# tyui592/Real_Time_Helmet_Detection

Hardware: AMD Instinct MI355X
Metric: train imgs/sec (higher is better)
Workload: dtype bf16; 1 GPU; model=hourglass-1-ch128, global_batch=16, imsize=512, parallelism=dp1, engine=hip, fp8=False, hipgraph=True

## Files before the change

### real_time_helmet_detection_amd/ops/csrc/bindings.cpp

```cpp
#include <torch/extension.h>

namespace rthd {
torch::Tensor add_act_fwd(torch::Tensor a, torch::Tensor b, int64_t act);
torch::Tensor add_act_bwd(torch::Tensor dy, torch::Tensor y, int64_t act);

std::vector<torch::Tensor> pool2x2_fwd(torch::Tensor x, bool is_max,
                                       bool need_arg);
torch::Tensor pool2x2_bwd(torch::Tensor dy, torch::Tensor arg, bool is_max,
                          int64_t H, int64_t W);
std::vector<torch::Tensor> maxpool_same_fwd(torch::Tensor x, int64_t k,
                                            bool need_arg);
torch::Tensor maxpool_same_bwd(torch::Tensor dy, torch::Tensor arg,
                               int64_t k);

torch::Tensor upsample2x_add_fwd(torch::Tensor x,
                                 c10::optional<torch::Tensor> skip);
torch::Tensor upsample2x_bwd(torch::Tensor dy);

std::vector<torch::Tensor> centernet_loss_fwd(
    torch::Tensor phm, torch::Tensor poff, torch::Tensor psize,
    torch::Tensor ghm, torch::Tensor goff, torch::Tensor gsize,
    torch::Tensor mask, double alpha, double beta);
std::vector<torch::Tensor> centernet_loss_bwd(
    torch::Tensor phm, torch::Tensor poff, torch::Tensor psize,
    torch::Tensor ghm, torch::Tensor goff, torch::Tensor gsize,
    torch::Tensor mask, torch::Tensor sums, torch::Tensor gout,
    double alpha, double beta);
std::vector<torch::Tensor> centernet_loss_fused_fwd(
    torch::Tensor out, torch::Tensor ghm, torch::Tensor goff,
    torch::Tensor gsize, torch::Tensor mask, double alpha, double beta,
    bool sig_os);
torch::Tensor centernet_loss_fused_bwd(
    torch::Tensor out, torch::Tensor ghm, torch::Tensor goff,
    torch::Tensor gsize, torch::Tensor mask, torch::Tensor sums,
    torch::Tensor glosses, double alpha, double beta, bool sig_os);

std::vector<torch::Tensor> decode_fwd(torch::Tensor hm, torch::Tensor off,
                                      torch::Tensor wh, int64_t scale_factor,
                                      int64_t topk, int64_t pool_size,
                                      bool normalized);
std::vector<torch::Tensor> decode_logits(torch::Tensor out,
                                         int64_t scale_factor, int64_t topk,
                                         int64_t pool_size, bool normalized,
                                         bool flip);
torch::Tensor nms_fwd(torch::Tensor boxes, torch::Tensor scores,
                      double iou_threshold);
std::vector<torch::Tensor> nms_batched(torch::Tensor boxes,
                                       torch::Tensor scores,
                                       double iou_threshold,
                                       double conf_th);
std::vector<torch::Tensor> soft_nms_fwd(torch::Tensor boxes,
                                        torch::Tensor scores, double sigma,
                                        double score_th);
std::vector<torch::Tensor> soft_nms_batched(torch::Tensor boxes,
                                            torch::Tensor scores,
                                            double sigma, double score_th,
                                            double conf_th);

torch::Tensor pack_weights(torch::Tensor w, bool swap, bool to_bf16);
std::vector<torch::Tensor> pack_weights_pair(torch::Tensor w,
                                             bool to_bf16_fwd,
                                             bool to_bf16_dgrad);
torch::Tensor pack_weights_fp8(torch::Tensor w);
torch::Tensor conv_fwd_fp8r(torch::Tensor x, torch::Tensor wpk,
                            torch::Tensor scale, torch::Tensor shift,
                            c10::optional<torch::Tensor> skip,
                            int64_t KH, int64_t KW, int64_t stride,
                            int64_t pad, int64_t Cout, int64_t act,
                            bool out_fp8);
torch::Tensor conv_fwd(torch::Tensor x, torch::Tensor wpk,
                       torch::Tensor scale, torch::Tensor shift,
                       c10::optional<torch::Tensor> skip,
                       int64_t KH, int64_t KW, int64_t stride, int64_t pad,
                       int64_t Cout, int64_t act);
torch::Tensor conv_fwd_small(torch::Tensor x, torch::Tensor wpk,
                             torch::Tensor scale, torch::Tensor shift,
                             c10::optional<torch::Tensor> skip,
                             int64_t KH, int64_t KW, int64_t stride,
                             int64_t pad, int64_t Cout, int64_t act,
                             int64_t splitk);
torch::Tensor conv_fwd_k64(torch::Tensor x, torch::Tensor wpk,
                           torch::Tensor scale, torch::Tensor shift,
                           c10::optional<torch::Tensor> skip,
                           int64_t KH, int64_t KW, int64_t stride,
                           int64_t pad, int64_t Cout, int64_t act);
torch::Tensor conv_fwd_halo(torch::Tensor x, torch::Tensor wpk,
                            torch::Tensor scale, torch::Tensor shift,
                            c10::optional<torch::Tensor> skip,
                            int64_t KH, int64_t KW, int64_t stride,
                            int64_t pad, int64_t Cout, int64_t act);
torch::Tensor stem_im2col(torch::Tensor x, int64_t KS, int64_t stride,
                          int64_t pad);
torch::Tensor wgrad(torch::Tensor x, torch::Tensor dy, int64_t KH,
                    int64_t KW, int64_t stride, int64_t pad);
torch::Tensor wgrad_bf16_fast(torch::Tensor x, torch::Tensor dy, int64_t KH,
                              int64_t KW, int64_t stride, int64_t pad,
                              const std::string& variant);
torch::Tensor lds_tr16_selftest();
std::string wgrad_bf16_choice(int64_t Cin, int64_t Cout, int64_t M);
int64_t wgrad_bf16_chunk_len(int64_t Cin, int64_t Cout, int64_t taps,
                             int64_t M);

std::vector<torch::Tensor> conv_fwd_stats(
    torch::Tensor x, torch::Tensor wpk, torch::Tensor scale,
    torch::Tensor shift, int64_t KH, int64_t KW, int64_t stride,
    int64_t pad, int64_t Cout, int64_t act);
std::vector<torch::Tensor> bn_stats_from_parts(
    torch::Tensor p1, torch::Tensor p2,
    c10::optional<torch::Tensor> running_mean,
    c10::optional<torch::Tensor> running_var,
    double momentum, double eps, int64_t M);
std::vector<torch::Tensor> bn_stats(torch::Tensor x,
                                    c10::optional<torch::Tensor> running_mean,
                                    c10::optional<torch::Tensor> running_var,
                                    double momentum, double eps);
torch::Tensor bn_act_fwd(torch::Tensor x, torch::Tensor mean,
                         torch::Tensor rstd, torch::Tensor gamma,
                         torch::Tensor beta, int64_t act,
                         c10::optional<torch::Tensor> skip);
std::vector<torch::Tensor> bn_act_bwd(torch::Tensor dy, torch::Tensor x,
                                      torch::Tensor mean, torch::Tensor rstd,
                                      torch::Tensor gamma, torch::Tensor beta,
                                      int64_t act,
                                      c10::optional<torch::Tensor> skip);
torch::Tensor col_sum(torch::Tensor x);

std::vector<torch::Tensor> encode_targets(torch::Tensor boxes,
                                          torch::Tensor labels, int64_t H,
                                          int64_t W, int64_t scale_factor,
                                          int64_t num_cls, bool normalized);
torch::Tensor normalize_u8(torch::Tensor img_u8, torch::Tensor table);
int64_t encode_chunk();
torch::Tensor augment_u8(torch::Tensor img_u8, torch::Tensor sizes,
                         torch::Tensor coef, int64_t T,
                         c10::optional<torch::Tensor> table);
}

PYBIND11_MODULE(TORCH_EXTENSION_NAME, m) {
  m.def("add_act_fwd", &rthd::add_act_fwd);
  m.def("add_act_bwd", &rthd::add_act_bwd);
  m.def("pool2x2_fwd", &rthd::pool2x2_fwd);
  m.def("pool2x2_bwd", &rthd::pool2x2_bwd);
  m.def("maxpool_same_fwd", &rthd::maxpool_same_fwd);
  m.def("maxpool_same_bwd", &rthd::maxpool_same_bwd);
  m.def("upsample2x_add_fwd", &rthd::upsample2x_add_fwd);
  m.def("upsample2x_bwd", &rthd::upsample2x_bwd);
  m.def("centernet_loss_fwd", &rthd::centernet_loss_fwd);
  m.def("centernet_loss_bwd", &rthd::centernet_loss_bwd);
  m.def("centernet_loss_fused_fwd", &rthd::centernet_loss_fused_fwd);
  m.def("centernet_loss_fused_bwd", &rthd::centernet_loss_fused_bwd);
  m.def("decode_fwd", &rthd::decode_fwd);
  m.def("decode_logits", &rthd::decode_logits);
  m.def("nms_fwd", &rthd::nms_fwd);
  m.def("nms_batched", &rthd::nms_batched);
  m.def("soft_nms", &rthd::soft_nms_fwd);
  m.def("soft_nms_batched", &rthd::soft_nms_batched);
  m.def("pack_weights",&rthd::pack_weights);
  m.def("pack_weights_pair", &rthd::pack_weights_pair);
  m.def("pack_weights_fp8", &rthd::pack_weights_fp8);
  m.def("conv_fwd_fp8r", &rthd::conv_fwd_fp8r);
  m.def("conv_fwd", &rthd::conv_fwd);
  m.def("conv_fwd_small", &rthd::conv_fwd_small);
  m.def("conv_fwd_k64", &rthd::conv_fwd_k64);
  m.def("conv_fwd_halo", &rthd::conv_fwd_halo);
  m.def("stem_im2col", &rthd::stem_im2col);
  m.def("wgrad", &rthd::wgrad);
  m.def("wgrad_bf16_fast", &rthd::wgrad_bf16_fast,
        py::arg("x"), py::arg("dy"), py::arg("kh"), py::arg("kw"),
        py::arg("stride"), py::arg("pad"), py::arg("variant") = "");
  m.def("lds_tr16_selftest", &rthd::lds_tr16_selftest);
  m.def("wgrad_bf16_choice", &rthd::wgrad_bf16_choice);
  m.def("wgrad_bf16_chunk_len", &rthd::wgrad_bf16_chunk_len);
  m.def("conv_fwd_stats", &rthd::conv_fwd_stats);
  m.def("bn_stats_from_parts", &rthd::bn_stats_from_parts,
        py::arg("p1"), py::arg("p2"), py::arg("running_mean") = py::none(),
        py::arg("running_var") = py::none(), py::arg("momentum") = 0.1,
        py::arg("eps") = 1e-5, py::arg("m") = 1);
  m.def("bn_stats", &rthd::bn_stats);
  m.def("bn_act_fwd", &rthd::bn_act_fwd, py::arg("x"), py::arg("mean"), py::arg("rstd"), py::arg("gamma"), py::arg("beta"), py::arg("act"), py::arg("skip") = py::none());
  m.def("bn_act_bwd", &rthd::bn_act_bwd, py::arg("dy"), py::arg("x"), py::arg("mean"), py::arg("rstd"), py::arg("gamma"), py::arg("beta"), py::arg("act"), py::arg("skip") = py::none());
  m.def("col_sum", &rthd::col_sum);
  m.def("encode_targets", &rthd::encode_targets);
  m.def("normalize_u8", &rthd::normalize_u8);
  m.def("encode_chunk", &rthd::encode_chunk);
  m.def("augment_u8", &rthd::augment_u8, py::arg("img_u8"), py::arg("sizes"),
        py::arg("coef"), py::arg("T"), py::arg("table") = py::none());
}

namespace rthd {

static torch::Tensor maxpool2x2_op(torch::Tensor x) {
  return pool2x2_fwd(std::move(x), true, false)[0];
}
static torch::Tensor avgpool2x2_op(torch::Tensor x) {
  return pool2x2_fwd(std::move(x), false, false)[0];
}
static torch::Tensor maxpool_same_op(torch::Tensor x, int64_t k) {
  return maxpool_same_fwd(std::move(x), k, false)[0];
}
static std::tuple<torch::Tensor, torch::Tensor> nms_batched_op(
    torch::Tensor boxes, torch::Tensor scores, double iou, double conf) {
  auto v = nms_batched(std::move(boxes), std::move(scores), iou, conf);
  return {v[0], v[1]};
}
static std::tuple<torch::Tensor, torch::Tensor> soft_nms_op(
    torch::Tensor boxes, torch::Tensor scores, double sigma,
    double score_th) {
  auto v = soft_nms_fwd(std::move(boxes), std::move(scores), sigma, score_th);
  return {v[0], v[1]};
}
static std::tuple<torch::Tensor, torch::Tensor, torch::Tensor>
soft_nms_batched_op(torch::Tensor boxes, torch::Tensor scores, double sigma,
                    double score_th, double conf) {
  auto v = soft_nms_batched(std::move(boxes), std::move(scores), sigma,
                            score_th, conf);
  return {v[0], v[1], v[2]};
}
static std::tuple<torch::Tensor, torch::Tensor, torch::Tensor> decode_op(
    torch::Tensor hm, torch::Tensor off, torch::Tensor wh,
    int64_t scale_factor, int64_t topk, int64_t pool_size, bool normalized) {
  auto v = decode_fwd(std::move(hm), std::move(off), std::move(wh),
                      scale_factor, topk, pool_size, normalized);
  return {v[0], v[1], v[2]};
}
static std::tuple<torch::Tensor, torch::Tensor, torch::Tensor>
decode_logits_op(torch::Tensor out, int64_t scale_factor, int64_t topk,
                 int64_t pool_size, bool normalized, bool flip) {
  auto v = decode_logits(std::move(out), scale_factor, topk, pool_size,
                         normalized, flip);
  return {v[0], v[1], v[2]};
}

}

TORCH_LIBRARY(rthd, m) {
  m.def("conv_fwd(Tensor x, Tensor wpk, Tensor scale, Tensor shift, "
        "Tensor? skip, int kh, int kw, int stride, int pad, int cout, "
        "int act) -> Tensor");
  m.def("conv_fwd_fp8r(Tensor x, Tensor wpk, Tensor scale, Tensor shift, "
        "Tensor? skip, int kh, int kw, int stride, int pad, int cout, "
        "int act, bool out_fp8) -> Tensor");
  m.def("add_act_fwd(Tensor a, Tensor b, int act) -> Tensor");
  m.def("maxpool2x2(Tensor x) -> Tensor");
  m.def("avgpool2x2(Tensor x) -> Tensor");
  m.def("maxpool_same(Tensor x, int k) -> Tensor");
  m.def("upsample2x_add(Tensor x, Tensor? skip) -> Tensor");
  m.def("nms(Tensor boxes, Tensor scores, float iou) -> Tensor");
  m.def("nms_batched(Tensor boxes, Tensor scores, float iou, float conf) "
        "-> (Tensor, Tensor)");
  m.def("soft_nms(Tensor boxes, Tensor scores, float sigma, "
        "float score_th) -> (Tensor, Tensor)");
  m.def("soft_nms_batched(Tensor boxes, Tensor scores, float sigma, "
        "float score_th, float conf) -> (Tensor, Tensor, Tensor)");
  m.def("decode(Tensor hm, Tensor off, Tensor wh, int scale_factor, "
        "int topk, int pool_size, bool normalized) "
        "-> (Tensor, Tensor, Tensor)");
  m.def("decode_logits(Tensor out, int scale_factor, int topk, "
        "int pool_size, bool normalized, bool flip) "
        "-> (Tensor, Tensor, Tensor)");
  m.def("stem_im2col(Tensor x, int ks, int stride, int pad) -> Tensor");
}

TORCH_LIBRARY_IMPL(rthd, CUDA, m) {
  m.impl("conv_fwd", rthd::conv_fwd);
  m.impl("conv_fwd_fp8r", rthd::conv_fwd_fp8r);
  m.impl("add_act_fwd", rthd::add_act_fwd);
  m.impl("maxpool2x2", rthd::maxpool2x2_op);
  m.impl("avgpool2x2", rthd::avgpool2x2_op);
  m.impl("maxpool_same", rthd::maxpool_same_op);
  m.impl("upsample2x_add", rthd::upsample2x_add_fwd);
  m.impl("nms", rthd::nms_fwd);
  m.impl("nms_batched", rthd::nms_batched_op);
  m.impl("soft_nms", rthd::soft_nms_op);
  m.impl("soft_nms_batched", rthd::soft_nms_batched_op);
  m.impl("decode", rthd::decode_op);
  m.impl("decode_logits", rthd::decode_logits_op);
  m.impl("stem_im2col", rthd::stem_im2col);
}
```

### real_time_helmet_detection_amd/ops/csrc/wgrad_fast.hip

```cpp
#include <torch/extension.h>
#include <ATen/cuda/CUDAContext.h>
#include "common.h"
#include "wgrad_tr_geo.h"

namespace rthd {

const bf16* zero_page_bf16(const torch::Tensor& like);
void wgrad_tr_launch(const WtrGeo& g, int nchunks, const bf16* x,
                     const bf16* dy, const bf16* zpage, float* dwp,
                     hipStream_t s);

using bf16x8 = __attribute__((ext_vector_type(8))) short;
using f32x4 = __attribute__((ext_vector_type(4))) float;

DEV_INLINE int wg_off(int row, int px8) {
  return row * 272 + ((px8 ^ ((row >> 3) & 7)) << 4);
}

struct WgradGeo2 {
  int B, H, W, Cin, Ho, Wo, Cout;
  int KH, KW, stride, pad;
  int M;
  int chunk_len;
  int ci_tiles, co_tiles, nchunks;
};

#define WGRAD_NUM_XCD 8

template <bool ALIGNED, bool SAME>
__global__ __launch_bounds__(256)
void wgrad_bf16_kernel(const bf16* __restrict__ x,
                       const bf16* __restrict__ dy,
                       float* __restrict__ dw, WgradGeo2 g) {
  const int t = blockIdx.z % (g.KH * g.KW);
  const int chunk = blockIdx.z / (g.KH * g.KW);
  const int ci0 = blockIdx.x * 64;
  const int co0 = blockIdx.y * 64;
  const int dyt = t / g.KW - g.pad;
  const int dxt = t % g.KW - g.pad;
  const int dtoff = dyt * g.W + dxt;

  const int tid = threadIdx.x;
  const int lane = tid & 63;
  const int wid = tid >> 6;
  const int wr = wid >> 1, wc = wid & 1;

  __shared__ __attribute__((aligned(16))) char smem[2 * 64 * 272];
  bf16* Xl = reinterpret_cast<bf16*>(smem);
  bf16* Yl = reinterpret_cast<bf16*>(smem + 64 * 272);

  f32x4 acc[2][2] = {};

  const int px_start = chunk * g.chunk_len;
  const int px_end = min(px_start + g.chunk_len, g.M);

  const bool stage_x = tid < 128;
  const int s_ci = (tid & 7) * 8;
  const int s_px = ((tid >> 3) & 15) * 8;

  const int HoWo = g.Ho * g.Wo;
  int mb = px_start + s_px;
  int bb = mb / HoWo;
  int rr = mb - bb * HoWo;
  int oy = rr / g.Wo;
  int ox = rr - oy * g.Wo;

  ushort r[8][8];

#define RTHD_WG_LOADX(p0_)                                                   \
  {                                                                          \
    int bj = bb, oyj = oy, oxj = ox;                                         \
    const int cbase = ci0 + s_ci;                                            \
    _Pragma("unroll") for (int j = 0; j < 8; ++j) {                          \
      const int m = (p0_) + s_px + j;                                        \
      uint4 v;                                                               \
      const int iy = oyj * g.stride + dyt;                                   \
      const int ix = oxj * g.stride + dxt;                                   \
      const bool val = m < px_end && iy >= 0 && iy < g.H && ix >= 0 &&       \
                       ix < g.W && cbase < g.Cin;                            \
      if (ALIGNED) {                                                         \
                        \
        const int64_t off = !val ? 0                                         \
            : SAME ? (int64_t)(m + dtoff) * g.Cin + cbase                    \
            : (((int64_t)bj * g.H + iy) * g.W + ix) * g.Cin + cbase;         \
        v = *reinterpret_cast<const uint4*>(x + off);                        \
        if (!val) v = uint4{0, 0, 0, 0};                                     \
      } else {                                                               \
        v = uint4{0, 0, 0, 0};                                               \
        if (val) {                                                           \
          const ushort* src = reinterpret_cast<const ushort*>(               \
              x + (((int64_t)bj * g.H + iy) * g.W + ix) * g.Cin + cbase);    \
          ushort tmp[8] = {};                                                \
          for (int e = 0; cbase + e < g.Cin; ++e) tmp[e] = src[e];           \
          v = *reinterpret_cast<const uint4*>(tmp);                          \
        }                                                                    \
      }                                                                      \
      *reinterpret_cast<uint4*>(r[j]) = v;                                   \
      if (++oxj >= g.Wo) {                                                   \
        oxj = 0;                                                             \
        if (++oyj >= g.Ho) { oyj = 0; ++bj; }                                \
      }                                                                      \
    }                                                                        \
  }

#define RTHD_WG_LOADY(p0_)                                                   \
  {                                                                          \
    const int cbase = co0 + s_ci;                                            \
    _Pragma("unroll") for (int j = 0; j < 8; ++j) {                          \
      const int m = (p0_) + s_px + j;                                        \
      uint4 v;                                                               \
      const bool val = m < px_end && cbase < g.Cout;                         \
      if (ALIGNED) {                                                         \
        const int64_t off = val ? (int64_t)m * g.Cout + cbase : 0;           \
        v = *reinterpret_cast<const uint4*>(dy + off);                       \
        if (!val) v = uint4{0, 0, 0, 0};                                     \
      } else {                                                               \
        v = uint4{0, 0, 0, 0};                                               \
        if (val) {                                                           \
          const ushort* src = reinterpret_cast<const ushort*>(               \
              dy + (int64_t)m * g.Cout + cbase);                             \
          ushort tmp[8] = {};                                                \
          for (int e = 0; cbase + e < g.Cout; ++e) tmp[e] = src[e];          \
          v = *reinterpret_cast<const uint4*>(tmp);                          \
        }                                                                    \
      }                                                                      \
      *reinterpret_cast<uint4*>(r[j]) = v;                                   \
    }                                                                        \
  }

  if (stage_x) RTHD_WG_LOADX(px_start) else RTHD_WG_LOADY(px_start)

  for (int p0 = px_start; p0 < px_end; p0 += 128) {
    __syncthreads();
    {
      bf16* half = stage_x ? Xl : Yl;
#pragma unroll
      for (int e = 0; e < 8; ++e) {
        ushort o[8];
#pragma unroll
        for (int j = 0; j < 8; ++j) o[j] = r[j][e];
        *reinterpret_cast<uint4*>(
            reinterpret_cast<char*>(half) +
            wg_off(s_ci + e, s_px >> 3)) = *reinterpret_cast<uint4*>(o);
      }
    }
    if (stage_x) {
      ox += 128;
      while (ox >= g.Wo) {
        ox -= g.Wo;
        if (++oy >= g.Ho) { oy = 0; ++bb; }
      }
    }
    __syncthreads();
    if (p0 + 128 < px_end) {
      if (stage_x) RTHD_WG_LOADX(p0 + 128) else RTHD_WG_LOADY(p0 + 128)
    }

    asm volatile("s_setprio 1");
#pragma unroll
    for (int ks = 0; ks < 4; ++ks) {
      const int k8 = (lane >> 4) + ks * 4;
      bf16x8 xa[2], yb[2];
#pragma unroll
      for (int i = 0; i < 2; ++i) {
        const int arow = wr * 32 + i * 16 + (lane & 15);
        xa[i] = *reinterpret_cast<const bf16x8*>(
            reinterpret_cast<char*>(Xl) + wg_off(arow, k8));
        const int brow = wc * 32 + i * 16 + (lane & 15);
        yb[i] = *reinterpret_cast<const bf16x8*>(
            reinterpret_cast<char*>(Yl) + wg_off(brow, k8));
      }
#pragma unroll
      for (int mi = 0; mi < 2; ++mi)
#pragma unroll
        for (int ni = 0; ni < 2; ++ni)
          acc[mi][ni] = __builtin_amdgcn_mfma_f32_16x16x32_bf16(
              xa[mi], yb[ni], acc[mi][ni], 0, 0, 0);
    }
    asm volatile("s_setprio 0");
  }

#undef RTHD_WG_LOADX
#undef RTHD_WG_LOADY

  const int ty = t / g.KW, tx = t % g.KW;
  float* dwc = dw + (int64_t)chunk * g.Cout * g.Cin * g.KH * g.KW;
#pragma unroll
  for (int mi = 0; mi < 2; ++mi) {
#pragma unroll
    for (int r2 = 0; r2 < 4; ++r2) {
      const int ci = ci0 + wr * 32 + mi * 16 + (lane >> 4) * 4 + r2;
      if (ci >= g.Cin) continue;
#pragma unroll
      for (int ni = 0; ni < 2; ++ni) {
        const int co = co0 + wc * 32 + ni * 16 + (lane & 15);
        if (co >= g.Cout) continue;
        dwc[(((int64_t)co * g.KH + ty) * g.KW + tx) * g.Cin + ci] =
            acc[mi][ni][r2];
      }
    }
  }
}

__global__ void wgrad_reduce_kernel(const float* __restrict__ part,
                                    float* __restrict__ out,
                                    int K, int64_t N) {
  const int64_t n4 = N >> 2;
  for (int64_t i = blockIdx.x * (int64_t)blockDim.x + threadIdx.x;
       i < n4; i += (int64_t)gridDim.x * blockDim.x) {
    float4 a = {0.f, 0.f, 0.f, 0.f};
    int k = 0;
    for (; k + 3 < K; k += 4) {
      float4 v[4];
#pragma unroll
      for (int u = 0; u < 4; ++u)
        v[u] = *reinterpret_cast<const float4*>(
            &part[(int64_t)(k + u) * N + i * 4]);
#pragma unroll
      for (int u = 0; u < 4; ++u) {
        a.x += v[u].x; a.y += v[u].y; a.z += v[u].z; a.w += v[u].w;
      }
    }
    for (; k < K; ++k) {
      const float4 v =
          *reinterpret_cast<const float4*>(&part[(int64_t)k * N + i * 4]);
      a.x += v.x; a.y += v.y; a.z += v.z; a.w += v.w;
    }
    *reinterpret_cast<float4*>(&out[i * 4]) = a;
  }
  for (int64_t i = n4 * 4 + blockIdx.x * (int64_t)blockDim.x + threadIdx.x;
       i < N; i += (int64_t)gridDim.x * blockDim.x) {
    float a = 0.f;
    for (int k = 0; k < K; ++k) a += part[(int64_t)k * N + i];
    out[i] = a;
  }
}

static bool wgrad_default_is_tr(int Cin, int Cout, int M) {
  constexpr int kTrMinPx = 4096;
  const char* e = getenv("RTHD_WGRAD_REGT");
  const bool force_regt = e && atoi(e) != 0;
  return Cin % 8 == 0 && Cout % 8 == 0 && !force_regt && M > kTrMinPx;
}

std::string wgrad_bf16_choice(int64_t Cin, int64_t Cout, int64_t M) {
  return wgrad_default_is_tr((int)Cin, (int)Cout, (int)M) ? "tr" : "regt";
}

int64_t wgrad_bf16_chunk_len(int64_t Cin, int64_t Cout, int64_t taps,
                             int64_t M) {
  int forced = 0;
  if (const char* e = getenv("RTHD_WGRAD_CHUNK")) forced = atoi(e);
  return wtr_chunk_len((int)M, (int)Cin, (int)Cout, (int)taps, forced);
}

torch::Tensor wgrad_bf16_fast(torch::Tensor x, torch::Tensor dy, int64_t KH,
                              int64_t KW, int64_t stride, int64_t pad,
                              const std::string& variant) {
  auto xc = x.contiguous(at::MemoryFormat::ChannelsLast);
  auto dyc = dy.to(at::kBFloat16).contiguous(at::MemoryFormat::ChannelsLast);
  WgradGeo2 g;
  g.B = xc.size(0);
  g.Cin = xc.size(1);
  g.H = xc.size(2);
  g.W = xc.size(3);
  g.Cout = dyc.size(1);
  g.Ho = dyc.size(2);
  g.Wo = dyc.size(3);
  g.KH = KH; g.KW = KW; g.stride = stride; g.pad = pad;
  g.M = g.B * g.Ho * g.Wo;

  const int ci_tiles = (int)cdiv(g.Cin, 64);
  const int co_tiles = (int)cdiv(g.Cout, 64);
  const int taps = (int)(KH * KW);
  const int chunk_len = (int)wgrad_bf16_chunk_len(g.Cin, g.Cout, taps, g.M);
  const int nchunks = (int)cdiv(g.M, chunk_len);
  g.chunk_len = chunk_len;
  g.ci_tiles = ci_tiles;
  g.co_tiles = co_tiles;
  g.nchunks = nchunks;

  const int64_t N = (int64_t)g.Cout * g.Cin * KH * KW;
  auto dwp = torch::empty({(int64_t)nchunks * N},
                          xc.options().dtype(at::kFloat));
  auto dw = torch::empty({g.Cout, g.Cin, KH, KW},
                         xc.options().dtype(at::kFloat).memory_format(
                             at::MemoryFormat::ChannelsLast));

  dim3 grid(ci_tiles, co_tiles, taps * nchunks);
  auto s = at::cuda::getCurrentCUDAStream();
  const bool aligned = (g.Cin % 8 == 0) && (g.Cout % 8 == 0);

  bool use_tr = false;
  if (variant == "tr") {
    TORCH_CHECK(aligned, "wgrad_bf16_fast: variant 'tr' needs Cin % 8 == 0 "
                "and Cout % 8 == 0");
    use_tr = true;
  } else if (variant.empty()) {
    use_tr = wgrad_default_is_tr(g.Cin, g.Cout, g.M);
  } else {
    TORCH_CHECK(variant == "regt", "wgrad_bf16_fast: unknown variant '",
                variant, "'");
  }
  const bool same = stride == 1 && g.Ho == g.H && g.Wo == g.W;
  auto* px = reinterpret_cast<const bf16*>(xc.data_ptr());
  auto* pdy = reinterpret_cast<const bf16*>(dyc.data_ptr());
#define RTHD_WG_LAUNCH(A_, S_)                                           \
  hipLaunchKernelGGL((wgrad_bf16_kernel<A_, S_>), grid, dim3(256), 0, s, \
      px, pdy, dwp.data_ptr<float>(), g)
  if (use_tr) {
    WtrGeo tg;
    tg.B = g.B; tg.H = g.H; tg.W = g.W; tg.Cin = g.Cin;
    tg.Ho = g.Ho; tg.Wo = g.Wo; tg.Cout = g.Cout;
    tg.KH = g.KH; tg.KW = g.KW; tg.stride = g.stride; tg.pad = g.pad;
    tg.M = g.M; tg.chunk_len = g.chunk_len;
    wgrad_tr_launch(tg, nchunks, px, pdy, zero_page_bf16(xc),
                    dwp.data_ptr<float>(), s);
  }
  else if (aligned && same) RTHD_WG_LAUNCH(true, true);
  else if (aligned)    RTHD_WG_LAUNCH(true, false);
  else if (same)       RTHD_WG_LAUNCH(false, true);
  else                 RTHD_WG_LAUNCH(false, false);
#undef RTHD_WG_LAUNCH
  const int rblocks = (int)std::min<int64_t>(2048, cdiv(N, 4 * 256) + 1);
  hipLaunchKernelGGL(wgrad_reduce_kernel, dim3(rblocks), dim3(256), 0, s,
      dwp.data_ptr<float>(), dw.data_ptr<float>(), nchunks, N);
  HIP_CHECK_LAST();
  return dw;
}

}
```

Baseline: 1279 imgs/sec.

## Add row-shared wgrad kernel reusing one x tile across three horizontal taps

Adds a new weight-gradient kernel for 3x3 stride-1 pad-1 convs. Each block stages one row-shifted x strip, with a one-pixel apron, plus a dy tile in LDS, and computes all three horizontal taps (dx = -1, 0, +1) from it. Edge columns are handled by masking the transposed LDS reads. This cuts x loads and the tap dimension of the grid by three compared with the per-tap 'tr' kernel, and it uses a triple-buffered global_load_lds pipeline. It becomes the default for large eligible shapes (M > 65536, channels >= 64), at the cost of extra LDS and complex correctness-sensitive masking logic.

```diff
diff --git a/real_time_helmet_detection_amd/ops/csrc/bindings.cpp b/real_time_helmet_detection_amd/ops/csrc/bindings.cpp
--- a/real_time_helmet_detection_amd/ops/csrc/bindings.cpp
+++ b/real_time_helmet_detection_amd/ops/csrc/bindings.cpp
@@ -98,6 +98,10 @@
                               const std::string& variant);
 torch::Tensor lds_tr16_selftest();
 std::string wgrad_bf16_choice(int64_t Cin, int64_t Cout, int64_t M);
+std::string wgrad_bf16_choice_geo(int64_t Cin, int64_t Cout, int64_t KH,
+                                  int64_t KW, int64_t stride, int64_t pad,
+                                  int64_t H, int64_t W, int64_t B);
+int64_t wgrad_row_chunk_len(int64_t Cin, int64_t Cout, int64_t M);
 int64_t wgrad_bf16_chunk_len(int64_t Cin, int64_t Cout, int64_t taps,
                              int64_t M);
 
@@ -171,6 +175,11 @@
   m.def("lds_tr16_selftest", &rthd::lds_tr16_selftest);
   m.def("wgrad_bf16_choice", &rthd::wgrad_bf16_choice);
   m.def("wgrad_bf16_chunk_len", &rthd::wgrad_bf16_chunk_len);
+  m.def("wgrad_bf16_choice_geo", &rthd::wgrad_bf16_choice_geo,
+        py::arg("cin"), py::arg("cout"), py::arg("kh"), py::arg("kw"),
+        py::arg("stride"), py::arg("pad"), py::arg("h"), py::arg("w"),
+        py::arg("b"));
+  m.def("wgrad_row_chunk_len", &rthd::wgrad_row_chunk_len);
   m.def("conv_fwd_stats", &rthd::conv_fwd_stats);
   m.def("bn_stats_from_parts", &rthd::bn_stats_from_parts,
         py::arg("p1"), py::arg("p2"), py::arg("running_mean") = py::none(),
diff --git a/real_time_helmet_detection_amd/ops/csrc/wgrad_fast.hip b/real_time_helmet_detection_amd/ops/csrc/wgrad_fast.hip
--- a/real_time_helmet_detection_amd/ops/csrc/wgrad_fast.hip
+++ b/real_time_helmet_detection_amd/ops/csrc/wgrad_fast.hip
@@ -1,7 +1,7 @@
 #include <torch/extension.h>
 #include <ATen/cuda/CUDAContext.h>
 #include "common.h"
-#include "wgrad_tr_geo.h"
+#include "wgrad_row_geo.h"
 
 namespace rthd {
 
@@ -9,6 +9,9 @@
 void wgrad_tr_launch(const WtrGeo& g, int nchunks, const bf16* x,
                      const bf16* dy, const bf16* zpage, float* dwp,
                      hipStream_t s);
+void wgrad_row_launch(const WtrGeo& g, int nchunks, const bf16* x,
+                      const bf16* dy, const bf16* zpage, float* dwp,
+                      hipStream_t s);
 
 using bf16x8 = __attribute__((ext_vector_type(8))) short;
 using f32x4 = __attribute__((ext_vector_type(4))) float;
@@ -247,11 +250,47 @@
   return wgrad_default_is_tr((int)Cin, (int)Cout, (int)M) ? "tr" : "regt";
 }
 
+static bool wgrad_default_is_row(const WtrGeo& g) {
+  constexpr int kRowMinPx = 65536;
+  const char* e = getenv("RTHD_WGRAD_ROW");
+  if (e && atoi(e) == 0) return false;
+  return wrow_eligible(g) && g.Cin >= 64 && g.Cout >= 64 &&
+         g.M > kRowMinPx && wgrad_default_is_tr(g.Cin, g.Cout, g.M);
+}
+
+static WtrGeo wgrad_geo(int64_t B, int64_t Cin, int64_t H, int64_t W,
+                        int64_t Cout, int64_t KH, int64_t KW, int64_t stride,
+                        int64_t pad) {
+  WtrGeo g;
+  g.B = (int)B; g.H = (int)H; g.W = (int)W; g.Cin = (int)Cin;
+  g.Cout = (int)Cout;
+  g.KH = (int)KH; g.KW = (int)KW; g.stride = (int)stride; g.pad = (int)pad;
+  g.Ho = (int)((H + 2 * pad - KH) / stride + 1);
+  g.Wo = (int)((W + 2 * pad - KW) / stride + 1);
+  g.M = g.B * g.Ho * g.Wo;
+  g.chunk_len = 0;
+  return g;
+}
+
+std::string wgrad_bf16_choice_geo(int64_t Cin, int64_t Cout, int64_t KH,
+                                  int64_t KW, int64_t stride, int64_t pad,
+                                  int64_t H, int64_t W, int64_t B) {
+  const WtrGeo g = wgrad_geo(B, Cin, H, W, Cout, KH, KW, stride, pad);
+  if (wgrad_default_is_row(g)) return "row";
+  return wgrad_bf16_choice(Cin, Cout, g.M);
+}
+
 int64_t wgrad_bf16_chunk_len(int64_t Cin, int64_t Cout, int64_t taps,
                              int64_t M) {
   int forced = 0;
   if (const char* e = getenv("RTHD_WGRAD_CHUNK")) forced = atoi(e);
   return wtr_chunk_len((int)M, (int)Cin, (int)Cout, (int)taps, forced);
+}
+
+int64_t wgrad_row_chunk_len(int64_t Cin, int64_t Cout, int64_t M) {
+  int forced = 0;
+  if (const char* e = getenv("RTHD_WGRAD_CHUNK")) forced = atoi(e);
+  return wrow_chunk_len((int)M, (int)Cin, (int)Cout, forced);
 }
 
 torch::Tensor wgrad_bf16_fast(torch::Tensor x, torch::Tensor dy, int64_t KH,
@@ -270,10 +309,36 @@
   g.KH = KH; g.KW = KW; g.stride = stride; g.pad = pad;
   g.M = g.B * g.Ho * g.Wo;
 
+  const bool aligned = (g.Cin % 8 == 0) && (g.Cout % 8 == 0);
+  WtrGeo tg;
+  tg.B = g.B; tg.H = g.H; tg.W = g.W; tg.Cin = g.Cin;
+  tg.Ho = g.Ho; tg.Wo = g.Wo; tg.Cout = g.Cout;
+  tg.KH = g.KH; tg.KW = g.KW; tg.stride = g.stride; tg.pad = g.pad;
+  tg.M = g.M;
+
+  bool use_tr = false, use_row = false;
+  if (variant == "row") {
+    TORCH_CHECK(wrow_eligible(tg), "wgrad_bf16_fast: variant 'row' needs a "
+                "3x3 stride-1 pad-1 conv with Wo % 32 == 0, Cin % 8 == 0 and "
+                "Cout % 8 == 0");
+    use_row = true;
+  } else if (variant == "tr") {
+    TORCH_CHECK(aligned, "wgrad_bf16_fast: variant 'tr' needs Cin % 8 == 0 "
+                "and Cout % 8 == 0");
+    use_tr = true;
+  } else if (variant.empty()) {
+    use_row = wgrad_default_is_row(tg);
+    use_tr = !use_row && wgrad_default_is_tr(g.Cin, g.Cout, g.M);
+  } else {
+    TORCH_CHECK(variant == "regt", "wgrad_bf16_fast: unknown variant '",
+                variant, "'");
+  }
+
   const int ci_tiles = (int)cdiv(g.Cin, 64);
   const int co_tiles = (int)cdiv(g.Cout, 64);
   const int taps = (int)(KH * KW);
-  const int chunk_len = (int)wgrad_bf16_chunk_len(g.Cin, g.Cout, taps, g.M);
+  int chunk_len = (int)wgrad_bf16_chunk_len(g.Cin, g.Cout, taps, g.M);
+  if (use_row) chunk_len = (int)wgrad_row_chunk_len(g.Cin, g.Cout, g.M);
   const int nchunks = (int)cdiv(g.M, chunk_len);
   g.chunk_len = chunk_len;
   g.ci_tiles = ci_tiles;
@@ -289,31 +354,17 @@
 
   dim3 grid(ci_tiles, co_tiles, taps * nchunks);
   auto s = at::cuda::getCurrentCUDAStream();
-  const bool aligned = (g.Cin % 8 == 0) && (g.Cout % 8 == 0);
-
-  bool use_tr = false;
-  if (variant == "tr") {
-    TORCH_CHECK(aligned, "wgrad_bf16_fast: variant 'tr' needs Cin % 8 == 0 "
-                "and Cout % 8 == 0");
-    use_tr = true;
-  } else if (variant.empty()) {
-    use_tr = wgrad_default_is_tr(g.Cin, g.Cout, g.M);
-  } else {
-    TORCH_CHECK(variant == "regt", "wgrad_bf16_fast: unknown variant '",
-                variant, "'");
-  }
   const bool same = stride == 1 && g.Ho == g.H && g.Wo == g.W;
   auto* px = reinterpret_cast<const bf16*>(xc.data_ptr());
   auto* pdy = reinterpret_cast<const bf16*>(dyc.data_ptr());
 #define RTHD_WG_LAUNCH(A_, S_)                                           \
   hipLaunchKernelGGL((wgrad_bf16_kernel<A_, S_>), grid, dim3(256), 0, s, \
       px, pdy, dwp.data_ptr<float>(), g)
-  if (use_tr) {
-    WtrGeo tg;
-    tg.B = g.B; tg.H = g.H; tg.W = g.W; tg.Cin = g.Cin;
-    tg.Ho = g.Ho; tg.Wo = g.Wo; tg.Cout = g.Cout;
-    tg.KH = g.KH; tg.KW = g.KW; tg.stride = g.stride; tg.pad = g.pad;
-    tg.M = g.M; tg.chunk_len = g.chunk_len;
+  tg.chunk_len = g.chunk_len;
+  if (use_row) {
+    wgrad_row_launch(tg, nchunks, px, pdy, zero_page_bf16(xc),
+                     dwp.data_ptr<float>(), s);
+  } else if (use_tr) {
     wgrad_tr_launch(tg, nchunks, px, pdy, zero_page_bf16(xc),
                     dwp.data_ptr<float>(), s);
   }
diff --git a/real_time_helmet_detection_amd/ops/csrc/wgrad_row.hip b/real_time_helmet_detection_amd/ops/csrc/wgrad_row.hip
--- /dev/null
+++ b/real_time_helmet_detection_amd/ops/csrc/wgrad_row.hip
@@ -0,0 +1,297 @@
+#include <mutex>
+
+#include "conv_common.h"
+#include "wgrad_row_geo.h"
+
+namespace rthd {
+
+namespace {
+
+using i16x4 = __attribute__((ext_vector_type(4))) short;
+using u32x2 = __attribute__((ext_vector_type(2))) uint32_t;
+typedef __attribute__((address_space(3))) char lds_char;
+
+constexpr int WROW_NBUF = 3;
+constexpr int WROW_NUM_XCD = 8;
+
+template <int OFF>
+DEV_INLINE i16x4 row_tr_read(uint32_t addr) {
+  i16x4 v;
+  asm volatile("ds_read_b64_tr_b16 %0, %1 offset:%2"
+               : "=v"(v) : "v"(addr), "n"(OFF) : "memory");
+  return v;
+}
+
+template <int REG>
+DEV_INLINE i16x4 row_mask(i16x4 v, uint32_t word) {
+  u32x2 u = __builtin_bit_cast(u32x2, v);
+  u[REG] &= word;
+  return __builtin_bit_cast(i16x4, u);
+}
+
+template <int BM, int BN>
+__global__ __launch_bounds__(256, 2)
+void wgrad_row_kernel(const bf16* __restrict__ x, const bf16* __restrict__ dy,
+                      const bf16* __restrict__ zpage, float* __restrict__ dw,
+                      WtrGeo g, int xcd_remap) {
+  constexpr int MI = BM / 32, NI = BN / 32;
+  constexpr int NP = (WROW_USED * BM * 2 + 1023) / 1024;
+  constexpr int XB = NP * 1024;
+  constexpr int YB = WTR_KB * BN * 2;
+  constexpr int STAGE = XB + YB;
+  constexpr int NXMAX = (NP + 3) / 4;
+  constexpr int NXMIN = NP / 4;
+  constexpr int NY = YB / 4096;
+  constexpr int KS = WTR_KB / 32;
+  constexpr int RD1 = 2 * (3 * MI + NI);
+  static_assert(KS == 2, "the fragment reads below are written for KS = 2");
+  static_assert(NXMAX - NXMIN <= 1, "two wait counts");
+  extern __shared__ __attribute__((aligned(16))) char smem[];
+
+  const int ci_t = (g.Cin + BM - 1) / BM, co_t = (g.Cout + BN - 1) / BN;
+  int cell = blockIdx.x;
+  if (xcd_remap) {
+    const int G = gridDim.x, k = cell % WROW_NUM_XCD, j = cell / WROW_NUM_XCD;
+    cell = k * (G / WROW_NUM_XCD) + min(k, G % WROW_NUM_XCD) + j;
+  }
+  const int z = cell / (ci_t * co_t);
+  const int ty = z % 3;
+  const int chunk = z / 3;
+  const int ci0 = (cell % ci_t) * BM;
+  const int co0 = (cell / ci_t % co_t) * BN;
+  const int dyt = ty - 1;
+
+  const int tid = threadIdx.x;
+  const int lane = tid & 63;
+  const int wid = __builtin_amdgcn_readfirstlane(tid >> 6);
+  const int wr = wid >> 1, wc = wid & 1;
+  const int nxw = (NP - wid + 3) / 4;
+
+  const int px_start = chunk * g.chunk_len;
+  const int px_end = min(px_start + g.chunk_len, g.M);
+  const int nsteps = (px_end - px_start + WTR_KB - 1) / WTR_KB;
+
+  WtrPix pix[NXMAX];
+  int xrow[NXMAX], xch[NXMAX], yrow[NY], ych[NY];
+#pragma unroll
+  for (int i = 0; i < NXMAX; ++i) {
+    int c;
+    wtr_stage_slot(i * 4 + wid, lane, BM, &xrow[i], &c);
+    xch[i] = ci0 + c * 8;
+    wrow_pix_init(px_start - WROW_APRON + xrow[i], g.Ho, g.Wo, &pix[i]);
+  }
+#pragma unroll
+  for (int i = 0; i < NY; ++i) {
+    int c;
+    wtr_stage_slot(i * 4 + wid, lane, BN, &yrow[i], &c);
+    ych[i] = co0 + c * 8;
+  }
+  const int adv_b = WTR_KB / (g.Ho * g.Wo);
+  const int adv_q = WTR_KB % (g.Ho * g.Wo) / g.Wo, adv_r = WTR_KB % g.Wo;
+
+  auto issue_step = [&](int step, int buf) {
+    char* base = smem + buf * STAGE;
+    const int p0 = px_start + step * WTR_KB;
+#pragma unroll
+    for (int i = 0; i < NXMAX; ++i) {
+      if (i < NXMIN || i < nxw) {
+        const int64_t off = wrow_x_src(g, pix[i], p0 - WROW_APRON + xrow[i],
+                                       xrow[i], px_end, dyt, xch[i]);
+        const bf16* src = off < 0 ? zpage : x + off;
+        __builtin_amdgcn_global_load_lds((glb_void*)src,
+            (lds_void*)(base + wtr_stage_byte(i * 4 + wid, lane)), 16, 0, 0);
+        wtr_pix_advance(&pix[i], adv_b, adv_q, adv_r, g.Ho, g.Wo);
+      }
+    }
+#pragma unroll
+    for (int i = 0; i < NY; ++i) {
+      const int64_t off = wtr_dy_src(g, p0 + yrow[i], px_end, ych[i]);
+      const bf16* src = off < 0 ? zpage : dy + off;
+      __builtin_amdgcn_global_load_lds((glb_void*)src,
+          (lds_void*)(base + XB + wtr_stage_byte(i * 4 + wid, lane)),
+          16, 0, 0);
+    }
+  };
+
+  const uint32_t lds0 = (uint32_t)(uintptr_t)(lds_char*)smem;
+  uint32_t aoff[3][MI][2], boff[NI][2];
+#pragma unroll
+  for (int h = 0; h < 2; ++h) {
+#pragma unroll
+    for (int t = 0; t < 3; ++t)
+#pragma unroll
+      for (int mi = 0; mi < MI; ++mi)
+        aoff[t][mi][h] =
+            lds0 + wrow_tr_addr(wr * MI + mi, 0, h, t - 1, lane, BM);
+#pragma unroll
+    for (int ni = 0; ni < NI; ++ni)
+      boff[ni][h] = lds0 + XB + wtr_tr_addr(wc * NI + ni, 0, h, lane, BN);
+  }
+  const uint32_t mword_lo = wrow_mask_word(-1, lane);
+  const uint32_t mword_hi = wrow_mask_word(+1, lane);
+  int oxs = __builtin_amdgcn_readfirstlane(px_start % g.Wo);
+
+  f32x4 acc[3][MI][NI] = {};
+
+  issue_step(0, 0);
+  if (nsteps > 1) issue_step(1, 1);
+  int rbuf = 0;
+
+  for (int step = 0; step < nsteps; ++step) {
+    if (step + 1 < nsteps) {
+      if (nxw == NXMAX)
+        asm volatile("s_waitcnt vmcnt(%0)" ::"n"(NXMAX + NY) : "memory");
+      else
+        asm volatile("s_waitcnt vmcnt(%0)" ::"n"(NXMIN + NY) : "memory");
+    } else {
+      asm volatile("s_waitcnt vmcnt(0)" ::: "memory");
+    }
+    __builtin_amdgcn_s_barrier();
+
+    const uint32_t boffs = (uint32_t)(rbuf * STAGE);
+    i16x4 xlo[KS][3][MI], xhi[KS][3][MI], ylo[KS][NI], yhi[KS][NI];
+#pragma unroll
+    for (int t = 0; t < 3; ++t)
+#pragma unroll
+      for (int mi = 0; mi < MI; ++mi) {
+        xlo[0][t][mi] = row_tr_read<0>(aoff[t][mi][0] + boffs);
+        xhi[0][t][mi] = row_tr_read<0>(aoff[t][mi][1] + boffs);
+      }
+#pragma unroll
+    for (int ni = 0; ni < NI; ++ni) {
+      ylo[0][ni] = row_tr_read<0>(boff[ni][0] + boffs);
+      yhi[0][ni] = row_tr_read<0>(boff[ni][1] + boffs);
+    }
+#pragma unroll
+    for (int t = 0; t < 3; ++t)
+#pragma unroll
+      for (int mi = 0; mi < MI; ++mi) {
+        xlo[1][t][mi] = row_tr_read<32 * BM * 2>(aoff[t][mi][0] + boffs);
+        xhi[1][t][mi] = row_tr_read<32 * BM * 2>(aoff[t][mi][1] + boffs);
+      }
+#pragma unroll
+    for (int ni = 0; ni < NI; ++ni) {
+      ylo[1][ni] = row_tr_read<32 * BN * 2>(boff[ni][0] + boffs);
+      yhi[1][ni] = row_tr_read<32 * BN * 2>(boff[ni][1] + boffs);
+    }
+
+    const int wbuf = rbuf == 0 ? 2 : rbuf - 1;
+    if (step + 2 < nsteps) issue_step(step + 2, wbuf);
+    rbuf = rbuf == 2 ? 0 : rbuf + 1;
+
+    uint32_t mlo[KS], mhi[KS];
+#pragma unroll
+    for (int ks = 0; ks < KS; ++ks) {
+      int oxk = oxs + 32 * ks;
+      oxk -= oxk >= g.Wo ? g.Wo : 0;
+      mlo[ks] = wrow_edge(-1, oxk, g.Wo) ? mword_lo : 0xffffffffu;
+      mhi[ks] = wrow_edge(+1, oxk, g.Wo) ? mword_hi : 0xffffffffu;
+    }
+    oxs += adv_r;
+    oxs -= oxs >= g.Wo ? g.Wo : 0;
+
+    __builtin_amdgcn_sched_barrier(0);
+    __builtin_amdgcn_s_setprio(1);
+#pragma unroll
+    for (int ks = 0; ks < KS; ++ks) {
+      static_assert(RD1 >= 15, "lgkmcnt(15) must cover k-block 0");
+      if (ks == 0)
+        asm volatile("s_waitcnt lgkmcnt(15)");
+      else
+        asm volatile("s_waitcnt lgkmcnt(0)");
+#pragma unroll
+      for (int t = 0; t < 3; ++t)
+#pragma unroll
+        for (int mi = 0; mi < MI; ++mi)
+          asm volatile("" : "+v"(xlo[ks][t][mi]), "+v"(xhi[ks][t][mi]));
+#pragma unroll
+      for (int ni = 0; ni < NI; ++ni)
+        asm volatile("" : "+v"(ylo[ks][ni]), "+v"(yhi[ks][ni]));
+      __builtin_amdgcn_sched_barrier(0);
+      bf16x8 yb[NI];
+#pragma unroll
+      for (int ni = 0; ni < NI; ++ni)
+        yb[ni] = __builtin_shufflevector(ylo[ks][ni], yhi[ks][ni], 0, 1, 2,
+                                         3, 4, 5, 6, 7);
+#pragma unroll
+      for (int t = 0; t < 3; ++t)
+#pragma unroll
+        for (int mi = 0; mi < MI; ++mi) {
+          i16x4 lo = xlo[ks][t][mi], hi = xhi[ks][t][mi];
+          if (t == 0) lo = row_mask<0>(lo, mlo[ks]);
+          if (t == 2) hi = row_mask<1>(hi, mhi[ks]);
+          const bf16x8 xa =
+              __builtin_shufflevector(lo, hi, 0, 1, 2, 3, 4, 5, 6, 7);
+#pragma unroll
+          for (int ni = 0; ni < NI; ++ni)
+            acc[t][mi][ni] = __builtin_amdgcn_mfma_f32_16x16x32_bf16(
+                xa, yb[ni], acc[t][mi][ni], 0, 0, 0);
+        }
+      __builtin_amdgcn_sched_barrier(0);
+    }
+    __builtin_amdgcn_s_setprio(0);
+    __builtin_amdgcn_sched_barrier(0);
+  }
+
+  float* dwc = dw + (int64_t)chunk * g.Cout * g.Cin * 9;
+#pragma unroll
+  for (int mi = 0; mi < MI; ++mi) {
+#pragma unroll
+    for (int r = 0; r < 4; ++r) {
+      const int ci = ci0 + (wr * MI + mi) * 16 + (lane >> 4) * 4 + r;
+      if (ci >= g.Cin) continue;
+#pragma unroll
+      for (int ni = 0; ni < NI; ++ni) {
+        const int co = co0 + (wc * NI + ni) * 16 + (lane & 15);
+        if (co >= g.Cout) continue;
+#pragma unroll
+        for (int t = 0; t < 3; ++t)
+          dwc[(((int64_t)co * 3 + ty) * 3 + t) * g.Cin + ci] =
+              acc[t][mi][ni][r];
+      }
+    }
+  }
+}
+
+template <int BM, int BN>
+void row_launch_tile(const WtrGeo& g, int nchunks, const bf16* x,
+                     const bf16* dy, const bf16* zpage, float* dwp,
+                     hipStream_t s) {
+  const dim3 grid((unsigned)(cdiv(g.Cin, BM) * cdiv(g.Cout, BN) * 3 *
+                             nchunks));
+  const int remap = g.M >= 65536;
+  const size_t lds =
+      (size_t)WROW_NBUF * (wrow_x_pieces(BM) * 1024 + WTR_KB * BN * 2);
+  {
+    static std::mutex mu;
+    static uint64_t done = 0;
+    int dev = 0;
+    TORCH_CHECK(hipGetDevice(&dev) == hipSuccess && dev < 64,
+                "wgrad_row: bad device");
+    std::lock_guard<std::mutex> lk(mu);
+    if (!((done >> dev) & 1)) {
+      const hipError_t e = hipFuncSetAttribute(
+          reinterpret_cast<const void*>(&wgrad_row_kernel<BM, BN>),
+          hipFuncAttributeMaxDynamicSharedMemorySize, (int)lds);
+      TORCH_CHECK(e == hipSuccess, "wgrad_row: cannot opt in to ", lds,
+                  " B of LDS: ", hipGetErrorString(e));
+      done |= (uint64_t)1 << dev;
+    }
+  }
+  hipLaunchKernelGGL((wgrad_row_kernel<BM, BN>), grid, dim3(256), lds, s, x,
+                     dy, zpage, dwp, g, remap);
+}
+
+}
+
+constexpr int WROW_BM = 64, WROW_BN = 128;
+
+void wgrad_row_launch(const WtrGeo& g, int nchunks, const bf16* x,
+                      const bf16* dy, const bf16* zpage, float* dwp,
+                      hipStream_t s) {
+  TORCH_CHECK(wrow_eligible(g) && g.chunk_len % 128 == 0,
+              "wgrad_row: ineligible shape");
+  row_launch_tile<WROW_BM, WROW_BN>(g, nchunks, x, dy, zpage, dwp, s);
+}
+
+}
diff --git a/real_time_helmet_detection_amd/ops/csrc/wgrad_row_geo.h b/real_time_helmet_detection_amd/ops/csrc/wgrad_row_geo.h
--- /dev/null
+++ b/real_time_helmet_detection_amd/ops/csrc/wgrad_row_geo.h
@@ -0,0 +1,71 @@
+#pragma once
+
+#include "wgrad_tr_geo.h"
+
+namespace rthd {
+
+constexpr int WROW_APRON = 1;
+constexpr int WROW_USED = WTR_KB + 2;
+
+WTR_HD int wrow_x_pieces(int CH) {
+  return (WROW_USED * CH * 2 + 1023) / 1024;
+}
+WTR_HD int wrow_x_rows(int CH) { return wrow_x_pieces(CH) * 1024 / (CH * 2); }
+
+WTR_HD int wrow_x_wave_pieces(int wid, int CH) {
+  return (wrow_x_pieces(CH) - wid + 3) / 4;
+}
+
+constexpr int WROW_BLOCKS = 512;
+
+WTR_HD int wrow_chunk_len(int M, int Cin, int Cout, int forced) {
+  const int tiles = ((Cin + 63) / 64) * ((Cout + 127) / 128) * 3;
+  const int nchunks = WROW_BLOCKS / tiles > 1 ? WROW_BLOCKS / tiles : 1;
+  int len = ((M + nchunks - 1) / nchunks + 127) / 128 * 128;
+  if (forced >= 128) len = (forced + 127) / 128 * 128;
+  return len;
+}
+
+WTR_HD bool wrow_eligible(const WtrGeo& g) {
+  return g.KH == 3 && g.KW == 3 && g.stride == 1 && g.pad == 1 &&
+         g.Ho == g.H && g.Wo == g.W && g.Wo % 32 == 0 && g.Cin % 8 == 0 &&
+         g.Cout % 8 == 0;
+}
+
+WTR_HD int wrow_tr_addr(int frag, int ks, int h, int dx, int lane, int CH) {
+  const int g = lane >> 4, q = (lane >> 2) & 3, p = lane & 3;
+  const int row = WROW_APRON + dx + 32 * ks + 8 * g + 4 * h + q;
+  return wtr_lds_off(row, 2 * frag + (p >> 1), CH) + 8 * (p & 1);
+}
+
+WTR_HD void wrow_pix_init(int m, int Ho, int Wo, WtrPix* p) {
+  if (m < 0) {
+    p->b = -1;
+    p->oy = Ho - 1;
+    p->ox = Wo + m;
+  } else {
+    wtr_pix_init(m, Ho, Wo, p);
+  }
+}
+
+WTR_HD int64_t wrow_x_src(const WtrGeo& g, const WtrPix& p, int m, int row,
+                          int px_end, int dyt, int c) {
+  const int iy = p.oy + dyt;
+  const bool ok = (row < WROW_USED) & (m >= 0) & (m < g.M) & (m <= px_end) &
+                  (iy >= 0) & (iy < g.H) & (c < g.Cin);
+  const int64_t off = (int64_t)((p.b * g.H + iy) * g.W + p.ox) * g.Cin + c;
+  return ok ? off : -1;
+}
+
+WTR_HD bool wrow_edge(int dx, int oxk, int Wo) {
+  return dx < 0 ? oxk == 0 : dx > 0 ? oxk + 32 == Wo : false;
+}
+WTR_HD int wrow_mask_half(int dx) { return dx > 0; }
+WTR_HD int wrow_mask_reg(int dx) { return dx > 0; }
+WTR_HD uint32_t wrow_mask_word(int dx, int lane) {
+  return dx < 0 ? (lane < 16 ? 0xffff0000u : 0xffffffffu)
+       : dx > 0 ? (lane >= 48 ? 0x0000ffffu : 0xffffffffu)
+                : 0xffffffffu;
+}
+
+}
```

Result: faster. 1327 imgs/sec (median of 6 runs) (+3.8%).
